# titus-leistner/mmlf

Measured on AMD Instinct MI355X. Metric: 96x96 EPI patches/sec fwd+bwd, bs=512, higher is better.
Workload: dtype f32 via 2 x f16 operand split (22 significant bits per operand, locally scaled; 3 MFMA passes, f32 accumulate)

## Files before the change

### include/mmlf_hip.h

```cpp
#ifndef MMLF_HIP_H
#define MMLF_HIP_H

#include <stddef.h>
#include <stdint.h>

#ifdef __cplusplus
extern "C" {
#endif

#define MMLF_TILE_POSITIONS 256

const char *mmlf_last_error(void);
#define MMLF_ABI_VERSION 10
int mmlf_abi_version(void);

const char *mmlf_build_info(void);
int mmlf_build_is_ablation(void);
int mmlf_conv_cus(void);

enum { MMLF_AUDIT_IN = 0, MMLF_AUDIT_PACKED = 1, MMLF_AUDIT_BIAS = 2, MMLF_AUDIT_OUT = 3, MMLF_AUDIT_REF = 4,
       MMLF_AUDIT_IN_AMAX = 5, MMLF_AUDIT_OUT_AMAX = 6, MMLF_AUDIT_BN_PARTIAL = 7, MMLF_AUDIT_MASK = 8, MMLF_AUDIT_CONV_N = 9 };
int mmlf_audit_conv_h2(int cs_in, int K, int N, int cs_out, int N_store, int out_shift, int cs_ref, int B, int H, int W,
                       int64_t *ends);
enum { MMLF_AUDIT_WG_IN = 0, MMLF_AUDIT_WG_G = 1, MMLF_AUDIT_WG_GW = 2, MMLF_AUDIT_WG_GB = 3, MMLF_AUDIT_WG_WORKSPACE = 4,
       MMLF_AUDIT_WG_IN_AMAX = 5, MMLF_AUDIT_WG_G_AMAX = 6, MMLF_AUDIT_WGRAD_N = 7 };
int mmlf_audit_wgrad_h2(int cs_in, int Cin, int cs_g, int Cout, int g_shift, int B, int H, int W, int64_t *ends);

int64_t mmlf_grid_alloc_positions(int B, int H, int W);
int64_t mmlf_packed_filter_floats(int K, int N);
int64_t mmlf_wgrad_workspace_floats(int Cin, int Cout, int B, int H, int W);

enum { MMLF_VAR_IDENTITY = 0, MMLF_VAR_TRANSPOSE = 1, MMLF_VAR_TRANSPOSE_FLIPH = 2 };

int mmlf_pack_filter(const float *w_oihw, float *packed, int Cout, int Cin, int variant, int dgrad,
                     void *stream);

int mmlf_conv2x2(const float *in, int cs_in, int K, const float *packed, const float *bias, int N,
                 float *out, int cs_out, int N_store, int out_shift, int vh, int vw,
                 int B, int H, int W, int relu, const float *relu_ref, int cs_ref, void *stream);

int64_t mmlf_packed_filter_split_bytes(int K, int N);
int mmlf_pack_filter_split(const float *w_oihw, void *packed, int Cout, int Cin, int variant, int dgrad,
                           void *stream);
int mmlf_conv2x2_split(const float *in, int cs_in, int K, const void *packed, const float *bias, int N,
                       float *out, int cs_out, int N_store, int out_shift, int vh, int vw,
                       int B, int H, int W, int relu, const float *relu_ref, int cs_ref, void *stream);
// ... 2 lines not shown
int mmlf_grid_pad_w(void);
int mmlf_grid_pad_h(void);
int mmlf_amax_head(void);
int mmlf_amax_shard_stride(void);
int64_t mmlf_packed_filter_h2_bytes(int K, int N);
int mmlf_pack_filter_h2(const float *w_oihw, void *packed, int Cout, int Cin, int variant, int dgrad, void *stream);
typedef struct mmlf_pack_desc {
    const float *w_oihw;
    void *packed;
    int32_t Cout, Cin, variant, dgrad;
    int32_t col0;
    int32_t np;
} mmlf_pack_desc;
int mmlf_packed_filter_h2_columns(int N);
int mmlf_pack_filters_h2(const mmlf_pack_desc *table, int n, int total_columns, void *stream);
int mmlf_conv2x2_h2(const float *in, int cs_in, int K, const void *packed, const float *bias, int N,
                    float *out, int cs_out, int N_store, int out_shift, int vh, int vw,
                    int B, int H, int W, int relu, const float *relu_ref, int cs_ref,
                    const float *in_amax , float *out_amax ,
                    double *bn_partial ,
                    uint32_t *relu_mask_out , const uint32_t *relu_mask_in , void *stream);
int64_t mmlf_relu_mask_words(int B, int H, int W);
int mmlf_conv2x2_blocks(int K, int N, int B, int H, int W);

int64_t mmlf_conv2x2_thin_workspace_floats(int B, int H, int W);
int mmlf_conv2x2_thin(const float *in, int cs_in, int K, const float *w_oihw, const float *bias, int N,
                      float *out, int cs_out, int out_shift, int vh, int vw, int B, int H, int W, int relu,
                      int variant, float *workspace, float *out_amax, void *stream);
int64_t mmlf_conv2x2_wgrad_thin_workspace_floats(int Cin);
int mmlf_conv2x2_wgrad_thin(const float *in, int cs_in, int Cin, const float *g, int cs_g, int Cout, int g_shift,
                            float *gw_oihw, float *gb, int variant, int accumulate, float *workspace,
                            int B, int H, int W, void *stream);

int mmlf_conv2x2_wgrad(const float *in, int cs_in, int Cin, const float *g, int cs_g, int Cout,
                       int g_shift, float *gw_oihw, float *gb, int variant, int accumulate,
                       float *workspace, int B, int H, int W, void *stream);

int mmlf_conv2x2_wgrad_split(const float *in, int cs_in, int Cin, const float *g, int cs_g, int Cout,
                             int g_shift, float *gw_oihw, float *gb, int variant, int accumulate,
                             float *workspace, int B, int H, int W, void *stream);

int mmlf_conv2x2_wgrad_h2(const float *in, int cs_in, int Cin, const float *g, int cs_g, int Cout,
                          int g_shift, float *gw_oihw, float *gb, int variant, int accumulate,
                          float *workspace, int B, int H, int W, const float *in_amax, const float *g_amax,
                          void *stream);

int mmlf_bn_stats_train(const float *z, int cs, int C, const float *gamma, const float *beta,
                        float *running_mean, float *running_var, double momentum, double eps,
                        float *save_mean, float *save_invstd, float *scale, float *shift,
                        double *partial, int nblocks, int B, int H, int W, void *stream);
int mmlf_bn_coeffs_eval(const float *gamma, const float *beta, const float *running_mean,
                        const float *running_var, double eps, float *scale, float *shift, int C,
                        void *stream);
int mmlf_fold_bn_eval(const float *w_oihw, const float *bias, const float *scale, const float *shift,
                      float *w_out, float *bias_out, int Cout, int Cin, void *stream);
int mmlf_bn_stats_finalize(const double *partial, int nblocks, int C, const float *gamma, const float *beta,
                           float *running_mean, float *running_var, double momentum, double eps,
                           float *save_mean, float *save_invstd, float *scale, float *shift,
                           int B, int H, int W, void *stream);
int mmlf_bn_apply_relu(const float *z, int cs_z, int C, const float *scale, const float *shift,
                       float *y, int cs_y, int c_off, int C_store, int B, int H, int W,
                       float *amax_out , void *stream);
int mmlf_bn_apply_relu4(const float *const z[4], int cs_z, int C, const float *const scale[4],
                        const float *const shift[4], float *y, int cs_y, int B, int H, int W,
                        float *amax_out , void *stream);
int mmlf_bn_bwd_reduce(const float *gy, int cs_gy, int c_off, const float *z, int cs_z, int C,
                       const float *scale, const float *shift, const float *gamma,
                       const float *save_mean, const float *save_invstd,
                       float *dgamma, float *dbeta, int accumulate, float *coef,
                       double *partial, int nblocks, int B, int H, int W, void *stream);
int mmlf_bn_bwd_apply(const float *gy, int cs_gy, int c_off, const float *z, int cs_z, int C,
                      const float *scale, const float *shift, const float *save_mean,
                      const float *coef, float *dz, int cs_dz, int B, int H, int W,
                      float *amax_out , void *stream);
int mmlf_relu_bwd_slice(const float *src, int cs_src, int c_off, const float *ref, int cs_ref, int ref_off, int C,
                        float *dst, int cs_dst, int B, int H, int W,
// ... 77 lines not shown
```

### mmlf_amd/csrc/wgrad.hip

```cpp
#include "conv_device.h"
#include "wgrad_map.h"
#include "row_walk.h"

#ifdef MMLF_BOUNDS_DEBUG
int mmlf_oob_counts_wgrad(unsigned long long *host8, int reset)
{
    if (hipMemcpyFromSymbol(host8, HIP_SYMBOL(g_mmlf_oob), sizeof(unsigned long long) * 8) != hipSuccess) return 1;
    if (reset) {
        const unsigned long long z[8] = {};
        if (hipMemcpyToSymbol(HIP_SYMBOL(g_mmlf_oob), z, sizeof(z)) != hipSuccess) return 1;
    }
    return 0;
}
#endif

struct WgradArgs {
    const float *in;
    const float *g;
    float *part;
    long long NQpad;
    int cs_in, cin, cs_g, g_shift, P, nsplit, nslice, chunks_per_split, nchunks;
    int items;
    int g_cols;
    const float *in_amax, *g_amax;
// ... 845 lines not shown
    WgradPlan p;
    if (!wgrad_plan(0, Cin, Cout, -1, p) || B <= 0 || H <= 0 || W <= 0) return -1;
    return p.scales_off + 2 * (make_grid(B, H, W).NQpad / WG_KQ) + 4;
}

template <int KS, int NT>
static int launch_wgrad_f32(const WgradArgs &a, hipStream_t st)
{
    using S = WgradF32Shape<KS>;
    const dim3 grid(wgrad_grid_blocks(a.nslice, a.nsplit)), block(64 * S::WAVES);
    if constexpr (KS == 2) hipLaunchKernelGGL(wgrad4tap_kernel<NT>, grid, block, S::lds_bytes(NT), st, a);
    else hipLaunchKernelGGL(wgrad9tap_kernel<NT>, grid, block, S::lds_bytes(NT), st, a);
    return mmlf_launch_status(KS == 2 ? "mmlf_conv2x2_wgrad" : "mmlf_conv3x3_wgrad");
}

template <int MB, int NB, int PL>
static int launch_wgrad16(const WgradArgs &a, hipStream_t st)
{
    constexpr size_t lds = 2 * PL * 34 * 32 * (MB | 1) + PL * WG_KQ * 32 * (NB | 1);
    static PerDeviceOnce attr_once;
    if (attr_once.run([] { return mmlf_allow_lds(reinterpret_cast<const void *>(wgrad4tap_x6n_kernel<MB, NB, PL>), lds, "mmlf_conv2x2_wgrad_split"); }))
        return 1;
    hipLaunchKernelGGL((wgrad4tap_x6n_kernel<MB, NB, PL>), dim3(wgrad_grid_blocks(a.nslice, a.nsplit)), dim3(256), lds, st, a);
    return mmlf_launch_status("mmlf_conv2x2_wgrad_split");
}

static bool wgrad_persist()
{
    static const bool on = [] { const char *e = getenv("MMLF_WGRAD_PERSIST"); return !e || atoi(e) != 0; }();
    return on;
}

template <int PL>
static int launch_wgrad_wide(const WgradArgs &a, hipStream_t st)
{
    constexpr size_t lds = 2 * (2 * PL * 34 * 32 * (3 | 1) + PL * WG_KQ * 32 * (18 | 1));
    static PerDeviceOnce attr_once;
    if (attr_once.run([] { return mmlf_allow_lds(reinterpret_cast<const void *>(wgrad4tap_x6w_kernel<3, 9, PL>), lds, "mmlf_conv2x2_wgrad_split(wide)"); }))
        return 1;
    hipLaunchKernelGGL((wgrad4tap_x6w_kernel<3, 9, PL>), dim3(wgrad_wide_grid(a.items, device_cus(), wgrad_persist())), dim3(512), lds, st, a);
    return mmlf_launch_status("mmlf_conv2x2_wgrad_split");
}

template <int PL>
static int launch_wgrad_split(const Wgrad16Cfg &c, const WgradArgs &a, hipStream_t st)
{
    switch (10 * c.mb + c.nb) {
    case 22: return launch_wgrad16<2, 2, PL>(a, st);
    case 52: return launch_wgrad16<5, 2, PL>(a, st);
    case 25: return launch_wgrad16<2, 5, PL>(a, st);
    case 55: return launch_wgrad16<5, 5, PL>(a, st);
    case 28: return launch_wgrad16<2, 8, PL>(a, st);
    case 38: return launch_wgrad16<3, 8, PL>(a, st);
    default: return launch_wgrad_wide<PL>(a, st);
    }
}

static WgradArgs wgrad_args(const float *in, int cs_in, int Cin, const float *g, int cs_g, int g_shift, float *workspace,
                            const Grid &gr, long long alloc, long long part_floats)
{
    WgradArgs a = {};
    a.in = in; a.g = g; a.part = workspace; a.NQpad = gr.NQpad;
    a.cs_in = cs_in; a.cin = Cin; a.cs_g = a.g_cols = cs_g; a.g_shift = g_shift; a.P = gr.P;
    a.in_bytes = alloc * cs_in * 4; a.g_bytes = alloc * cs_g * 4;
    a.part_floats = part_floats;
    a.nchunks = (int)(gr.NQpad / WG_KQ);
    return a;
}
static void wgrad_set_grid(WgradArgs &a, int nslice, int nsplit)
{
    a.nslice = nslice;
    a.nsplit = nsplit;
    a.chunks_per_split = (a.nchunks + nsplit - 1) / nsplit;
    a.items = (int)wgrad_grid_blocks(nslice, nsplit);
}

template <int KS>
static int wgrad_reduce(const WgradArgs &a, float *gw, float *gb, int Cin, int Cout, int CIP, int NP, int variant,
                        int accumulate, hipStream_t st)
{
    const int total = KS * KS * (Cin + 1) * Cout;
    hipLaunchKernelGGL(wgrad_reduce_kernel<KS * KS>, dim3((total + 255) / 256), dim3(256), 0, st, a.part, gw, gb, Cin, Cout,
                       CIP, NP, a.nsplit, variant, accumulate);
    return mmlf_launch_status(KS == 2 ? "mmlf_conv2x2_wgrad(reduce)" : "mmlf_conv3x3_wgrad(reduce)");
}

template <int KS>
static int wgrad_run_block(WgradArgs &a, const WgradBlock &k, int planes, float *gw, float *gb, int Cin, int variant,
                           int accumulate, hipStream_t st)
{
    wgrad_set_grid(a, k.nslice, k.nsplit);
    int rc = 1;
    if constexpr (KS == 2) {
        if (!k.nt) rc = planes == 3 ? launch_wgrad_split<3>(k.cfg, a, st) : launch_wgrad_split<2>(k.cfg, a, st);
    }
    if (k.nt) switch (k.nt) {
    case 1: rc = launch_wgrad_f32<KS, 1>(a, st); break;
    case 3: rc = launch_wgrad_f32<KS, 3>(a, st); break;
    case 4: rc = launch_wgrad_f32<KS, 4>(a, st); break;
    default: rc = launch_wgrad_f32<KS, 9>(a, st); break;
    }
    if (rc) return rc;
    return wgrad_reduce<KS>(a, gw, gb, Cin, k.cout, k.CIP, k.NP, variant, accumulate, st);
}

static int wgrad_impl(const float *in, int cs_in, int Cin, const float *g, int cs_g, int Cout, int g_shift,
                      float *gw, float *gb, int variant, int accumulate, float *workspace, int B, int H, int W,
                      void *stream, int planes, const float *in_amax = nullptr, const float *g_amax = nullptr);

extern "C" int mmlf_conv2x2_wgrad(const float *in, int cs_in, int Cin, const float *g, int cs_g, int Cout,
                                  int g_shift, float *gw, float *gb, int variant, int accumulate,
                                  float *workspace, int B, int H, int W, void *stream)
{
    return wgrad_impl(in, cs_in, Cin, g, cs_g, Cout, g_shift, gw, gb, variant, accumulate, workspace, B, H, W,
                      stream, 0);
}

extern "C" int mmlf_conv2x2_wgrad_split(const float *in, int cs_in, int Cin, const float *g, int cs_g, int Cout,
                                        int g_shift, float *gw, float *gb, int variant, int accumulate,
                                        float *workspace, int B, int H, int W, void *stream)
{
    return wgrad_impl(in, cs_in, Cin, g, cs_g, Cout, g_shift, gw, gb, variant, accumulate, workspace, B, H, W,
                      stream, 3);
}

extern "C" int mmlf_conv2x2_wgrad_h2(const float *in, int cs_in, int Cin, const float *g, int cs_g, int Cout,
                                     int g_shift, float *gw, float *gb, int variant, int accumulate,
                                     float *workspace, int B, int H, int W, const float *in_amax,
                                     const float *g_amax, void *stream)
{
    MMLF_CHECK_ARG(in_amax && g_amax, "mmlf_conv2x2_wgrad_h2: the f16 split needs max |in| and max |g|");
    return wgrad_impl(in, cs_in, Cin, g, cs_g, Cout, g_shift, gw, gb, variant, accumulate, workspace, B, H, W,
                      stream, 2, in_amax, g_amax);
}

static int wgrad_impl(const float *in, int cs_in, int Cin, const float *g, int cs_g, int Cout, int g_shift,
                      float *gw, float *gb, int variant, int accumulate, float *workspace, int B, int H, int W,
                      void *stream, int planes, const float *in_amax, const float *g_amax)
{
    MMLF_CHECK_ARG(in && g && (gw || gb) && workspace, "mmlf_conv2x2_wgrad: null pointer");
    MMLF_CHECK_ARG(cs_in % 4 == 0 && cs_g % 4 == 0, "mmlf_conv2x2_wgrad: strides must be multiples of 4");
    MMLF_CHECK_ARG(Cin > 0 && Cin <= cs_in && Cout > 0 && Cout <= cs_g, "mmlf_conv2x2_wgrad: channels vs strides");
    MMLF_CHECK_ARG(Cout <= WGRAD_MAX_COUT_WIDE, "mmlf_conv2x2_wgrad: Cout=%d not supported (max %d)", Cout, WGRAD_MAX_COUT_WIDE);
    MMLF_CHECK_ARG(variant >= 0 && variant <= 2, "mmlf_conv2x2_wgrad: bad variant");
    Grid gr = make_grid(B, H, W);
    MMLF_CHECK_ARG(g_shift >= 0 && g_shift <= gr.P + 1, "mmlf_conv2x2_wgrad: g_shift=%d", g_shift);
    WgradPlan p;
    MMLF_CHECK_ARG(wgrad_plan(planes, Cin, Cout, gr.NQpad / WG_KQ, p), "mmlf_conv2x2_wgrad: no launch plan");
    WgradArgs a = wgrad_args(in, cs_in, Cin, g, cs_g, g_shift, workspace, gr, grid_alloc_positions(gr), p.scales_off);
    a.in_amax = in_amax; a.g_amax = g_amax;
    hipStream_t st = (hipStream_t)stream;
    if (!gw)
        return bias_grad_only("mmlf_conv2x2_wgrad", g, cs_g, Cout, g_shift, gb, accumulate, workspace, p.scales_off, gr, st);
    if (planes == 2) {
        MMLF_CHECK_ARG(gr.NQpad + 2 * gr.P + 64 < (1ll << 31), "mmlf_conv2x2_wgrad_h2: batch x image too large");
        ChunkScaleArgs ca;
        ca.in_amax = in_amax; ca.g_amax = g_amax; ca.out = workspace + p.scales_off;
        ca.NQ = gr.NQ; ca.nchunks = a.nchunks; ca.P = gr.P; ca.g_shift = g_shift;
        ca.nrows = (int)amax_rows(gr);
        ca.divP = make_magic((unsigned)gr.P);
        hipLaunchKernelGGL(wgrad_chunk_scales_kernel, dim3((a.nchunks + 255) / 256), dim3(256), 0, st, ca);
        a.chunk_scales = ca.out;
    }
    const WgradArgs whole = a;
    for (int b = 0; b < p.nblocks; ++b) {
        const int c0 = p.blk[b].c0;
        a = whole;
        a.g = g + c0; a.g_cols = cs_g - c0; a.g_bytes = whole.g_bytes - 4ll * c0;
        const int rc = wgrad_run_block<2>(a, p.blk[b], planes, gw + (size_t)c0 * Cin * 4, gb ? gb + c0 : nullptr, Cin, variant,
                                          accumulate, st);
        if (rc) return rc;
    }
    return 0;
}

__global__ __launch_bounds__(256) void thin_wgrad_kernel(ThinArgs a)
{
    const int lane = threadIdx.x & 63;
    const long long wave = __builtin_amdgcn_readfirstlane((int)(blockIdx.x * 4 + (threadIdx.x >> 6)));
    const long long nwaves = gridDim.x * 4ll;
    float acc[2][4][THIN_MAXN][4];
#pragma unroll
    for (int h = 0; h < 2; ++h)
#pragma unroll
        for (int t = 0; t < 4; ++t)
#pragma unroll
            for (int o = 0; o < THIN_MAXN; ++o)
#pragma unroll
                for (int k = 0; k < 4; ++k) acc[h][t][o][k] = 0.f;
    float gsum[THIN_MAXN] = {0.f, 0.f};
    const bool first = 4 * lane < a.cs_in, second = 256 + 4 * lane < a.cs_in;
    const int offs[4] = {0, 1, a.P, a.P + 1};
    constexpr int U = 4;
    for (long long p0 = U * wave; p0 < a.npos; p0 += U * nwaves) {
        float4 x0[U], x1[U];
        float gt[U][4][THIN_MAXN];
#pragma unroll
        for (int u = 0; u < U; ++u) {
            const long long p = p0 + u < a.npos ? p0 + u : a.npos - 1;
            const float *row = a.in + (size_t)p * a.cs_in;
            x0[u] = first ? *reinterpret_cast<const float4 *>(row + 4 * lane) : make_float4(0.f, 0.f, 0.f, 0.f);
            x1[u] = second ? *reinterpret_cast<const float4 *>(row + 256 + 4 * lane) : make_float4(0.f, 0.f, 0.f, 0.f);
#pragma unroll
// ... 140 lines not shown
```

### mmlf_amd/csrc/wgrad_map.h

```cpp
#pragma once

__host__ __device__ __forceinline__ bool wgrad_block_map(int b, int nslice, int nsplit, int &slice, int &split)
{
    const int x = b & 7, j = b >> 3;
    const int reg = (nsplit >> 3) * nslice;
    if (j < reg) {
        slice = j % nslice;
        split = (j / nslice) * 8 + x;
        return true;
    }
    const int left = (nsplit & 7) * nslice, per = (left + 7) >> 3;
    const int m = x * per + (j - reg);
    slice = m % nslice;
    split = (nsplit & ~7) + m / nslice;
    return m < left;
}

static inline unsigned wgrad_grid_blocks(int nslice, int nsplit)
{
    return 8u * (unsigned)((nsplit >> 3) * nslice + ((nsplit & 7) * nslice + 7) / 8);
}

static inline void wgrad_wide_splits(int Cin, long long nchunks, int cus, int &nslice, int &nsplit)
{
    nslice = (Cin + 1 + 47) / 48;
    if (cus > 256 || nchunks < 0) cus = 256;
    const int one_round = cus / nslice, three_rounds = (768 / nslice + 7) / 8 * 8;
    nsplit = nchunks < 0 ? (one_round > three_rounds ? one_round : three_rounds)
                         : (nchunks >= 42 * 1024 ? three_rounds : one_round);
    if (nsplit < 8) nsplit = 8;
}

static inline unsigned wgrad_wide_grid(int items, int cus, bool persist)
{
    if (!persist) return (unsigned)items;
    int resident = cus / 8 * 8;
    if (resident < 8) resident = 8;
    return (unsigned)(items < resident ? items : resident);
}
```

### mmlf_amd/engine.py

```python
import contextlib
import ctypes
import os
import threading
from collections import namedtuple

import torch

from . import _lib
from ._lib import call, check, ptr

VAR_IDENTITY, VAR_TRANSPOSE, VAR_TRANSPOSE_FLIPH = 0, 1, 2
BN_BLOCKS = 1024
LOSS_BLOCKS = 1024


MAX_WIDTH = {2: 512, 3: 288}
MAX_OC = 288
MAX_OVERLAP_WIDTH = 288


def cs_of(c):
    return (c + 7) // 8 * 8


# ... 168 lines not shown
def _toc(events, tag, flops, nbytes):
    events[1].record()
    PROFILE.append((tag, flops, events[0], events[1], nbytes))


@contextlib.contextmanager
def _timed(tag, flops, nbytes):
    events = _tic()
    yield
    _toc(events, tag, flops, nbytes)


_UNTIMED = contextlib.nullcontext()


def _amax_of(geo, t, cs):
    a = getattr(t, 'absmax', None)
    if a is None:
        return geo.amax_of(t, cs)
    if CHECK_ABSMAX:
        true = geo.amax_of(t, cs)
        c = geo.amax_canonical(a)
        exact = geo.P >= 32
        bad = (c != true) if exact else (c < true)
        bad[0] = c[0] != true[0]
        if bool(bad.any()):
            k = int(bad.nonzero()[0])
            raise AssertionError(f'amax entry {k} holds {float(c[k])!r}, true max |x| is {float(true[k])!r}')
    return a


CHECK_ABSMAX = bool(os.environ.get('MMLF_CHECK_ABSMAX'))
OVERLAP_WGRAD = os.environ.get('MMLF_OVERLAP_WGRAD', '1') not in ('', '0')


CHECK_EXTENTS = bool(os.environ.get('MMLF_CHECK_EXTENTS'))
EXTENT_CHECKS = 0


def _audit(entry, scalars, n_ends, kind, have):
    global EXTENT_CHECKS
    ends = (ctypes.c_int64 * n_ends)()
    call(entry, *scalars, ends)
    for name, (k, t, off) in have.items():
        if t is None:
            continue
        got = t.untyped_storage().nbytes() - t.storage_offset() * t.element_size() - 4 * off
        if ends[k] > got:
            raise RuntimeError(f'MMLF_CHECK_EXTENTS: {kind}: the launch may touch {ends[k]} bytes behind `{name}`, '
                               f'the tensor has {got}')
    EXTENT_CHECKS += 1


def relu_bwd_slice(geo, src, cs_src, c_off, ref, cs_ref, ref_off, C, dst, cs_dst):
    amax = getattr(dst, 'absmax', None)
    if CHECK_EXTENTS:
        _audit('mmlf_audit_relu_bwd_slice', (cs_src, c_off, cs_ref, ref_off, C, cs_dst, geo.B, geo.H, geo.W), 4,
               f'relu_bwd_slice C={C} {cs_src}+{c_off} B={geo.B} {geo.H}x{geo.W}',
               {'src': (0, src, 0), 'ref': (1, ref, 0), 'dst': (2, dst, 0), 'amax': (3, amax, 0)})
    call('mmlf_relu_bwd_slice', ptr(src), cs_src, c_off, ptr(ref), cs_ref, ref_off, C, ptr(dst), cs_dst, geo.B, geo.H, geo.W,
         ptr(amax), _lib.stream_ptr())


THIN_MAX_N, THIN_MIN_K = 2, 64


def wgrad(geo, x, cs_in, cin, g, cs_g, cout, g_shift, gw, gb, variant, workspace, side=False):
    if cout <= THIN_MAX_N and cin >= THIN_MIN_K and cs_in <= 512:
        ws = _Workspace.get(x.device).scratch('thin_wgrad', int(_lib.load().mmlf_conv2x2_wgrad_thin_workspace_floats(cin)), side)
        call('mmlf_conv2x2_wgrad_thin', ptr(x), cs_in, cin, ptr(g), cs_g, cout, g_shift, ptr(gw), ptr(gb), variant, 1,
             ptr(ws), geo.B, geo.H, geo.W, _lib.stream_ptr())
        return
    args = (ptr(x), cs_in, cin, ptr(g), cs_g, cout, g_shift, ptr(gw), ptr(gb), variant, 1, ptr(workspace),
            geo.B, geo.H, geo.W)
    timed = _UNTIMED
    if PROFILE is not None and cin >= 256 and cout >= 256 and gw is not None:
        vh, vw = (geo.H + 1, geo.W + 1) if g_shift == 0 else (geo.H, geo.W)
        nbytes = 4.0 * geo.B * (cin * (geo.H * geo.W if g_shift == 0 else (geo.H + 1) * (geo.W + 1)) + cout * vh * vw)
        timed = _timed('wgrad_side' if side else 'wgrad', 2.0 * geo.B * vh * vw * cout * 4 * cin, nbytes)
    with timed:
        if CONV_MODE == 'f16x3':
            ax, ag = _amax_of(geo, x, cs_in), _amax_of(geo, g, cs_g)
            if CHECK_EXTENTS:
                _audit('mmlf_audit_wgrad_h2', (cs_in, cin, cs_g, cout, g_shift, geo.B, geo.H, geo.W), 7,
                       f'wgrad {cin}->{cout} B={geo.B} {geo.H}x{geo.W} g_shift={g_shift}',
                       {'in': (0, x, 0), 'g': (1, g, 0), 'gw': (2, gw, 0), 'gb': (3, gb, 0), 'workspace': (4, workspace, 0),
                        'in_amax': (5, ax, 0), 'g_amax': (6, ag, 0)})
            call('mmlf_conv2x2_wgrad_h2', *args, ptr(ax), ptr(ag), _lib.stream_ptr())
        else:
            call('mmlf_conv2x2_wgrad_split' if CONV_MODE == 'bf16x6' else 'mmlf_conv2x2_wgrad', *args, _lib.stream_ptr())


def conv(geo, x, cs_in, K, packed, bias, N, out, cs_out, out_shift, vh, vw, relu, ref=None, cs_ref=0,
         n_store=None, out_off=0, bn_partial=None, mask_out=None, mask_in=None, w_master=None, variant=0):
    aout = getattr(out, 'absmax', None)
    if (w_master is not None and N <= THIN_MAX_N and K >= THIN_MIN_K and cs_in <= 512 and ref is None and mask_in is None
            and mask_out is None and bn_partial is None and out_off == 0 and n_store in (None, cs_out)):
        ws = _Workspace.get(x.device).scratch('thin_fwd', int(_lib.load().mmlf_conv2x2_thin_workspace_floats(geo.B, geo.H, geo.W)))
        call('mmlf_conv2x2_thin', ptr(x), cs_in, K, ptr(w_master), ptr(bias), N, ptr(out), cs_out, out_shift, vh, vw,
             geo.B, geo.H, geo.W, int(relu), variant, ptr(ws), ptr(aout), _lib.stream_ptr())
        return
    n_store = cs_out if n_store is None else n_store
    timed = _UNTIMED
    if PROFILE is not None and ((K >= 256 and N >= 256) or (K == N and 64 <= K < 128)):
        nbytes = 4.0 * geo.B * (K * (geo.H * geo.W if out_shift == 0 else (geo.H + 1) * (geo.W + 1)) + N * vh * vw)
        timed = _timed('conv' if K >= 256 else 'conv70', 2.0 * geo.B * vh * vw * N * 4 * K, nbytes)
# ... 67 lines not shown
    def __init__(self, geo, device, p=None, train=False, fold=False, plan=None, packs=None, sites=0, running=True):
        self.geo, self.device, self.p, self.train, self.fold, self.plan, self.running = geo, device, p, train, fold, plan, running
        self.packs, self.tracked, self.deferred, self.concat, self.recs = packs or {}, [], None, None, [None] * sites


class _SideWgrad:
    __slots__ = ('main', 'side', 'pending', 'kept', 'on_done')

    def __init__(self, ws, on_done, enabled):
        self.side = ws.side if enabled else None
        self.main = torch.cuda.current_stream() if self.side is not None else None
        self.pending, self.kept, self.on_done = None, None, on_done

    def takes(self, cin):
        return self.side is not None and 128 <= cin <= MAX_OVERLAP_WIDTH

    def launch(self, key, keep, run):
        ready = self.main.record_event()
        with torch.cuda.stream(self.side):
            self.side.wait_event(ready)
            run()
            self.pending, self.kept = (self.side.record_event(), key), keep

    def settle(self):
        if self.pending is not None:
            self.main.wait_event(self.pending[0])
            if self.on_done:
                self.on_done(self.pending[1])
            self.pending = None

    def done(self, key):
        if self.on_done and (self.pending is None or self.pending[1] != key):
            self.on_done(key)


class BlockPlan:
    LAUNCHES = ('reduce', 'apply', 'wgrad2', 'dgrad2', 'wgrad1', 'dgrad1')
    __slots__ = ('prefix', 'want') + LAUNCHES

    def __init__(self, prefix, want, bn, train, need_dx):
        self.prefix, self.want = prefix, frozenset(want)
        want_bn = bn and bool(self.want & {'3.weight', '3.bias'})
        self.wgrad1 = bool(self.want & {'0.weight', '0.bias'})
        self.wgrad2 = bool(self.want & {'2.weight', '2.bias'})
        self.dgrad1 = bool(need_dx)
        self.dgrad2 = self.wgrad1 or self.dgrad1
        need_dz = self.wgrad2 or self.dgrad2
        self.apply = bool(bn) and need_dz
        self.reduce = bool(bn) and (want_bn or (need_dz and bool(train)))

    def launches(self):
        return [k for k in self.LAUNCHES if getattr(self, k)]

    def __eq__(self, other):
        return isinstance(other, BlockPlan) and all(getattr(self, k) == getattr(other, k) for k in self.__slots__)

    def __repr__(self):
        return f'BlockPlan({self.prefix}: {" ".join(self.launches())}; {sorted(self.want)})'


class Plan:

    def __init__(self, trainable, input_grads, train, fold, streams, out, relu_only):
        self.trainable, self.input_grads, self.train, self.fold = trainable, input_grads, train, fold
        self.streams, self.out = streams, out
        self.stream_live = [any(b is not None for b in blocks) for blocks in streams]
# ... 120 lines not shown
                add(f'{spec.prefix}.0.weight', var, True)
        return _Workspace.get(dev).packed_filters(items)

    def _pack(self, w, var, dgrad):
        return (pack_filter3 if self.ksize == 3 else pack_filter)(w, var, dgrad)

    def _packed(self, tape, name, var, dgrad):
        pk = tape.packs.get((name, var, dgrad))
        return pk if pk is not None else self._pack(tape.p[name], var, dgrad)

    def _f16(self):
        return CONV_MODE == 'f16x3' and self.ksize == 2

    _extent = (lambda geo: (0, geo.H + 1, geo.W + 1), lambda geo: (geo.P + 1, geo.H, geo.W))

    def _conv(self, geo, x, f, out, off=None, stats=None):
        n_store, out_off = (out.cs, 0) if off is None else (f.N, off)
        if self.ksize == 3:
            assert out.mask is None and stats is None and f.master is None, (f, out.mask, stats)
            conv3(geo, x.t, x.cs, f.K, f.packed, f.bias, f.N, out.t, out.cs, out.relu, n_store=n_store, out_off=out_off)
            return
        conv(geo, x.t, x.cs, f.K, f.packed, f.bias, f.N, out.t, out.cs, *self._extent[f.second](geo), out.relu,
             n_store=n_store, out_off=out_off, bn_partial=stats, mask_out=out.mask, w_master=f.master, variant=f.var)

    def _dgrad(self, geo, g, f, dx, x):
        relu = {}
        if x.relu:
            relu = {'mask_in': x.mask} if x.mask is not None and self._f16() else {'ref': x.t, 'cs_ref': x.cs}
        if self.ksize == 3:
            conv3(geo, g.t, g.cs, f.N, f.packed, None, f.K, dx.t, dx.cs, False, **relu)
            return
        conv(geo, g.t, g.cs, f.N, f.packed, None, f.K, dx.t, dx.cs, *self._extent[not f.second](geo), False, **relu)

    def _wgrad(self, geo, f, x, g, into, side=False):
        ws = _Workspace.get(x.t.device).wgrad_ws(geo, f.K, f.N, side=side)
        if self.ksize == 3:
            wgrad3(geo, x.t, x.cs, f.K, g.t, g.cs, f.N, *into, f.var, ws)
        else:
            wgrad(geo, x.t, x.cs, f.K, g.t, g.cs, f.N, geo.P + 1 if f.second else 0, *into, f.var, ws, side=side)

    def _bn_fwd(self, tape, spec, z, rec):
        geo, p, pre, C, sp = tape.geo, tape.p, spec.prefix, spec.cout, _lib.stream_ptr
        coef = torch.empty((2 if z is None else 4) * C, dtype=torch.float32, device=tape.device)
        scale, shift = coef[:C], coef[C:2 * C]
        smean, sinv = (None, None) if z is None else (coef[2 * C:3 * C], coef[3 * C:])
        g, bt, rm, rv = (p[f'{pre}.3.{k}'] for k in ('weight', 'bias', 'running_mean', 'running_var'))
        if tape.train:
            partial = _Workspace.get(tape.device).partial
            moved = (rm, rv) if tape.running else (None, None)
            if self._f16():
                nblk = int(_lib.load().mmlf_conv2x2_blocks(C, C, geo.B, geo.H, geo.W))
                call('mmlf_bn_stats_finalize', ptr(partial), nblk, C, ptr(g), ptr(bt), ptr(moved[0]), ptr(moved[1]),
                     self.momentum, self.eps, ptr(smean), ptr(sinv), ptr(scale), ptr(shift), geo.B, geo.H, geo.W, sp())
            else:
                call('mmlf_bn_stats_train', ptr(z), cs_of(C), C, ptr(g), ptr(bt), ptr(moved[0]), ptr(moved[1]), self.momentum,
                     self.eps, ptr(smean), ptr(sinv), ptr(scale), ptr(shift), ptr(partial), BN_BLOCKS, geo.B, geo.H, geo.W, sp())
            if tape.running:
                tape.tracked.append(p[f'{pre}.3.num_batches_tracked'])
        else:
            call('mmlf_bn_coeffs_eval', ptr(g), ptr(bt), ptr(rm), ptr(rv), self.eps, ptr(scale), ptr(shift), C, sp())
            if rec is not None:
                smean.copy_(rm)
                sinv.copy_(torch.rsqrt(rv.double() + self.eps).float())
                rec.eval = True
        if rec is not None:
            rec.scale, rec.shift, rec.smean, rec.sinv = scale, shift, smean, sinv
        return scale, shift, smean, sinv

    def _block_fwd(self, tape, site, x, dest=None):
        geo, p, dev, spec, var = tape.geo, tape.p, tape.device, site.spec, site.var
        C, cs_mid, pre = spec.cout, cs_of(spec.cout), spec.prefix
        w1, b1, w2, b2 = p[f'{pre}.0.weight'], p[f'{pre}.0.bias'], p[f'{pre}.2.weight'], p[f'{pre}.2.bias']
# ... 101 lines not shown
                counts.setdefault(t.data_ptr(), [t, 0])[1] += 1
            torch._foreach_add_([t for t, _ in counts.values()], [n for _, n in counts.values()])
        out = torch.empty((B, self.oc, H, W), dtype=torch.float32, device=dev)
        call('mmlf_unpack_nchw', ptr(x.t), x.cs, ptr(out), self.oc, B, H, W, _lib.stream_ptr())
        if not (save and any(plan.slices)):
            tape.concat = None
        return out, (tape if save else None)

    def _bn_bwd(self, tape, rec, bp, grads, g, dz):
        geo, p, pre, C = tape.geo, tape.p, rec.spec.prefix, rec.spec.cout
        cs_mid, sp, ws = cs_of(C), _lib.stream_ptr, _Workspace.get(tape.device)
        g3w, g3b = (grads[f'{pre}.{k}'] if k in bp.want else None for k in ('3.weight', '3.bias'))
        coef = None
        if bp.reduce:
            coef = torch.empty(3 * C, dtype=torch.float32, device=tape.device)
            dgb = ws.scratch('bn_dgamma_dbeta', 2 * C) if g3w is None or g3b is None else None
            dgamma, dbeta = (dgb[:C] if g3w is None else g3w), (dgb[C:2 * C] if g3b is None else g3b)
            acc = int(g3w is not None or g3b is not None)
            call('mmlf_bn_bwd_reduce', ptr(g.t), g.cs, g.off, ptr(rec.z), cs_mid, C, ptr(rec.scale), ptr(rec.shift),
                 ptr(p[f'{pre}.3.weight']), ptr(rec.smean), ptr(rec.sinv), ptr(dgamma), ptr(dbeta), acc, ptr(coef),
                 ptr(ws.partial), BN_BLOCKS, geo.B, geo.H, geo.W, sp())
            if rec.eval and bp.apply:
                coef[C:].zero_()
        elif bp.apply:
            assert rec.eval, (pre, bp)
            coef = torch.zeros(3 * C, dtype=torch.float32, device=tape.device)
            coef[:C].copy_((p[f'{pre}.3.weight'].double() * rec.sinv.double()).float())
        if not bp.apply:
            return None, coef
        call('mmlf_bn_bwd_apply', ptr(g.t), g.cs, g.off, ptr(rec.z), cs_mid, C, ptr(rec.scale), ptr(rec.shift),
             ptr(rec.smean), ptr(coef), ptr(dz), cs_mid, geo.B, geo.H, geo.W, ptr(dz.absmax), sp())
        return _Slice(dz, cs_mid, 0), coef

    def _block_bwd(self, tape, rec, bp, grads, g, side=None):
        if rec is None:
            raise ValueError(f'Trunk.backward: the forward pass kept no record of {bp.prefix} (its trainable= / '
                             'input_grads= did not ask for what this backward needs)')
        spec, var, x, y, geo = rec.spec, rec.var, rec.x, rec.y, tape.geo
        C, cs_mid, pre = spec.cout, cs_of(spec.cout), spec.prefix
        assert not bp.want or rec.pk2d is None, 'a frozen forward (BatchNorm folded) has no parameter gradients'
        assert bool(rec.bn) or not (bp.reduce or bp.apply), (pre, bp)
        need_dx = bp.dgrad1
        gw1, gb1, gw2, gb2 = (grads[f'{pre}.{k}'] if k in bp.want else None for k in ('0.weight', '0.bias', '2.weight', '2.bias'))
        conv1, conv2 = _Filter(False, spec.cin, C, var), _Filter(True, C, C, var)
        css = ([cs_mid] if bp.apply else []) + ([cs_mid] if bp.dgrad2 else []) + ([x.cs] if need_dx else [])
        got = geo.bufs(css, tape.device) if css else []
        dy = _Slice(got[1 if bp.apply else 0], cs_mid, 0) if bp.dgrad2 else None
        dx = _Slice(got[-1], x.cs, 0) if need_dx else None
        if rec.bn:
            dz, coef = self._bn_bwd(tape, rec, bp, grads, g, got[0] if bp.apply else None)
        else:
            assert g.off == 0 and g.cs == cs_mid
            dz = g
        if side is not None:
            side.settle()
        if bp.wgrad2:
            self._wgrad(geo, conv2, y, dz, (gw2, gb2))
        if bp.dgrad2:
            pk2d = rec.pk2d if rec.pk2d is not None else self._packed(tape, f'{pre}.2.weight', var, True)
            self._dgrad(geo, dz, conv2._replace(packed=pk2d), dy, y)
        del dz, got
        overlap = side is not None and side.takes(spec.cin) and need_dx and bp.wgrad1
        if bp.wgrad1 and not overlap:
            self._wgrad(geo, conv1, x, dy, (gw1, gb1))
        if need_dx:
            self._dgrad(geo, dy, conv1._replace(packed=self._packed(tape, f'{pre}.0.weight', var, True)), dx, x)
        if overlap:
            side.launch(pre, (x.t, dy.t), lambda: self._wgrad(geo, conv1, x, dy, (gw1, gb1), side=True))
        elif side is not None:
            side.kept = None
        return dx

    def backward(self, p, tape, grad_output, grads, on_done=None, input_grads=None, packed_grads=False):
        geo, dev = tape.geo, tape.device
        check(grad_output, 'grad_output', dev, shape=(geo.B, self.oc, geo.H, geo.W), contiguous=False)
        fplan = tape.plan
        if grads is not None:
            wanted = self._grad_names if fplan is None else [n for n in self._grad_names if n in fplan.trainable]
            self._check_dict('grads', grads, wanted, dev)
        ws = _Workspace.get(dev)
        ws.enter_stream()
        B, H, W = geo.B, geo.H, geo.W
        g = _Slice(geo.buf(cs_of(self.oc), dev), cs_of(self.oc), 0)
        call('mmlf_pack_nchw', ptr(grad_output.contiguous()), self.oc, ptr(g.t), g.cs, B, H, W, ptr(g.t.absmax),
             _lib.stream_ptr())
        want = [bool(w) for w in input_grads] if input_grads is not None else [False] * 4
        assert len(want) == 4
        bplan = self.plan(fplan.trainable if grads is not None else (), want, fplan.train, fplan.fold)
        tape.p = p
        side =_SideWgrad(ws, on_done, OVERLAP_WGRAD and self.ksize == 2)
        dstacks = [None] * 4
        for site in reversed(self.sites):
            rec, tape.recs[site.index] = tape.recs[site.index], None
            bp, s = bplan.of(site), site.chain
            if s == 4:
                if bp is None:
                    g = None
                    side.settle()
                else:
                    g = self._block_bwd(tape, rec, bp, grads, g, side)
                side.done(site.spec.prefix)
                continue
            if site.last:
                if s == 2:
                    side.settle()
                gs = None if g is None else _Slice(g.t, g.cs, s * self.chs)
                if bplan.slices[s]:
                    if tape.concat is None:
                        raise ValueError('Trunk.backward: the forward pass kept no concat buffer for this backward')
                    gs = _Slice(geo.buf(cs_of(self.chs), dev), cs_of(self.chs), 0)
                    relu_bwd_slice(geo, g.t, g.cs, s * self.chs, tape.concat, g.cs, s * self.chs, self.chs, gs.t, gs.cs)
            if bp is not None:
                gs = self._block_bwd(tape, rec, bp, grads, gs)
            if site.k == 0:
                if want[s] and packed_grads:
                    assert gs.off == 0
                    dstacks[s] = (gs.t, gs.cs)
                elif want[s]:
                    dstacks[s] = torch.empty((B, self.views, 3, H, W), dtype=torch.float32, device=dev)
                    call('mmlf_unpack_nchw', ptr(gs.t), gs.cs, ptr(dstacks[s]), 3 * self.views, B, H, W, _lib.stream_ptr())
                if s in (2, 0):
                    side.done('in_net_id' if s == 2 else 'in_net_hv')
        tape.concat = None
        return dstacks
```

### mmlf_amd/train.py

```python
import math
import operator

import torch
import torch.distributed as dist

from . import _lib, dl, loss as loss_mod
from ._lib import call, ptr


def flatten_parameters(model):
    params = list(model.named_parameters())
    dev = params[0][1].device
    total = sum(p.numel() for _, p in params)
    flat = torch.empty(total, dtype=torch.float32, device=dev)
    layout, o = [], 0
    for name, p in params:
        n = p.numel()
        flat[o:o + n].copy_(p.detach().reshape(-1))
        p.data = flat[o:o + n].view_as(p)
        layout.append((name, o, n))
        o += n
    return flat, layout


# ... 339 lines not shown
        parts = [t.chunk(self.micro_batches) for t in tensors]
        if len(parts[0]) == 1:
            return None
        assert all(len(part) == len(parts[0]) for part in parts), [t.shape[0] for t in tensors]
        return list(zip(*parts))

    def _chunked_fwd_bwd(self, fwd_bwd, chunks, gt, mask, den):
        share = self.loss.chunks(len(chunks), self.micro_batches, gt, mask, den)
        losses, saved = [], None
        buffers = list(self.model.buffers()) if fwd_bwd == self._torch_fwd_bwd and self.model.training else []
        for k, chunk in enumerate(chunks):
            share.index = k
            losses.append(fwd_bwd(*chunk, share.den, share))
            if buffers:
                with torch.no_grad():
                    if saved is None:
                        saved = [b.clone() for b in buffers]
                    else:
                        torch._foreach_copy_(buffers, saved)
        return torch.stack(losses).sum()

    def _native_fwd_bwd(self, h, v, i_, d, gt, mask, den, share=None):
        model = self.model
        p = model._tensor_dict()
        with torch.no_grad():
            extra = {} if share is None else {'update_running': share.first(), 'packs': share.packs}
            out, tape = model._trunk.forward(p, [h, v, i_, d], model.training, True, trainable=self.trainable, **extra)
            den = self._den_end(den)
            if share is not None:
                share.den, share.packs = den, tape.packs
            loss, gout = self.loss.native(out, gt, mask, den, share)
            hooked = self.distributed and (share is None or share.last())
            on_done = (lambda key: self.buckets.ready(self.grad, key)) if hooked else None
            model._trunk.backward(p, tape, gout, self._trainable_grads or None, on_done)
        return loss

    def _torch_fwd_bwd(self, h, v, i_, d, gt, mask, den, share=None):
        model = self.model
        if share is None or share.first():
            for _, p in model.named_parameters():
                p.grad = None
        out = model(h, v, i_, d)
        den = self._den_end(den)
        if share is not None:
            share.den = den
        loss = self.loss.torch(out, gt, mask, den, share)
        loss.backward()
        if share is not None and not share.last():
            return loss.detach()
        for name, p in model.named_parameters():
            if p.grad is not None:
                self._grads[name].copy_(p.grad)
            p.grad = None
        return loss.detach()

    def _adam(self, lr, grad_scale):
        b1, b2 = self.betas
        t = self.adam_steps
        if self.flat.is_cuda:
            call('mmlf_adam_step', ptr(self.flat), ptr(self.grad), ptr(self.exp_avg), ptr(self.exp_avg_sq),
                 self.flat.numel(), lr, b1, b2, self.eps, t, grad_scale, _lib.stream_ptr())
            return
        with torch.no_grad():
            g = self.grad * grad_scale
            self.exp_avg.lerp_(g, 1 - b1)
            self.exp_avg_sq.mul_(b2).addcmul_(g, g, value=1 - b2)
            bc1, bc2 = 1 - b1 ** t, 1 - b2 ** t
# ... 24 lines not shown
```

Before: 1145.

## Defer chain-4 wgrads to side stream with a CU budget, overlapping the trunk backward

Weight-gradient launches for the first blocks of the shared chain-4 trunk are collected during backward. They are then replayed together on the side stream once the block's dgrad is issued, overlapping with the later backward work. A new flags field carries a CU budget that caps the persistent wide-wgrad grid, so the deferred kernels leave CUs free for the main stream. This adds stream/event synchronisation and a changed ABI, and only turns on in non-distributed training above a batch-size threshold, where the chosen budget may starve or oversubscribe either stream.

```diff
diff --git a/include/mmlf_hip.h b/include/mmlf_hip.h
--- a/include/mmlf_hip.h
+++ b/include/mmlf_hip.h
@@ -11,7 +11,7 @@
 #define MMLF_TILE_POSITIONS 256
 
 const char *mmlf_last_error(void);
-#define MMLF_ABI_VERSION 10
+#define MMLF_ABI_VERSION 11
 int mmlf_abi_version(void);
 
 const char *mmlf_build_info(void);
@@ -80,16 +80,20 @@
                             float *gw_oihw, float *gb, int variant, int accumulate, float *workspace,
                             int B, int H, int W, void *stream);
 
+#define MMLF_WGRAD_ACCUMULATE 1
+#define MMLF_WGRAD_BUDGET_SHIFT 8
+#define MMLF_WGRAD_BUDGET_MASK 0x00ffff00
+#define MMLF_WGRAD_BUDGET(cus) (((cus) << MMLF_WGRAD_BUDGET_SHIFT) & MMLF_WGRAD_BUDGET_MASK)
 int mmlf_conv2x2_wgrad(const float *in, int cs_in, int Cin, const float *g, int cs_g, int Cout,
-                       int g_shift, float *gw_oihw, float *gb, int variant, int accumulate,
+                       int g_shift, float *gw_oihw, float *gb, int variant, int flags,
                        float *workspace, int B, int H, int W, void *stream);
 
 int mmlf_conv2x2_wgrad_split(const float *in, int cs_in, int Cin, const float *g, int cs_g, int Cout,
-                             int g_shift, float *gw_oihw, float *gb, int variant, int accumulate,
+                             int g_shift, float *gw_oihw, float *gb, int variant, int flags,
                              float *workspace, int B, int H, int W, void *stream);
 
 int mmlf_conv2x2_wgrad_h2(const float *in, int cs_in, int Cin, const float *g, int cs_g, int Cout,
-                          int g_shift, float *gw_oihw, float *gb, int variant, int accumulate,
+                          int g_shift, float *gw_oihw, float *gb, int variant, int flags,
                           float *workspace, int B, int H, int W, const float *in_amax, const float *g_amax,
                           void *stream);
 
diff --git a/mmlf_amd/csrc/wgrad.hip b/mmlf_amd/csrc/wgrad.hip
--- a/mmlf_amd/csrc/wgrad.hip
+++ b/mmlf_amd/csrc/wgrad.hip
@@ -901,18 +901,18 @@
 }
 
 template <int PL>
-static int launch_wgrad_wide(const WgradArgs &a, hipStream_t st)
+static int launch_wgrad_wide(const WgradArgs &a, int budget, hipStream_t st)
 {
     constexpr size_t lds = 2 * (2 * PL * 34 * 32 * (3 | 1) + PL * WG_KQ * 32 * (18 | 1));
     static PerDeviceOnce attr_once;
     if (attr_once.run([] { return mmlf_allow_lds(reinterpret_cast<const void *>(wgrad4tap_x6w_kernel<3, 9, PL>), lds, "mmlf_conv2x2_wgrad_split(wide)"); }))
         return 1;
-    hipLaunchKernelGGL((wgrad4tap_x6w_kernel<3, 9, PL>), dim3(wgrad_wide_grid(a.items, device_cus(), wgrad_persist())), dim3(512), lds, st, a);
+    hipLaunchKernelGGL((wgrad4tap_x6w_kernel<3, 9, PL>), dim3(wgrad_wide_grid(a.items, wgrad_wide_budget_cus(device_cus(), budget), wgrad_persist())), dim3(512), lds, st, a);
     return mmlf_launch_status("mmlf_conv2x2_wgrad_split");
 }
 
 template <int PL>
-static int launch_wgrad_split(const Wgrad16Cfg &c, const WgradArgs &a, hipStream_t st)
+static int launch_wgrad_split(const Wgrad16Cfg &c, const WgradArgs &a, int budget, hipStream_t st)
 {
     switch (10 * c.mb + c.nb) {
     case 22: return launch_wgrad16<2, 2, PL>(a, st);
@@ -921,7 +921,7 @@
     case 55: return launch_wgrad16<5, 5, PL>(a, st);
     case 28: return launch_wgrad16<2, 8, PL>(a, st);
     case 38: return launch_wgrad16<3, 8, PL>(a, st);
-    default: return launch_wgrad_wide<PL>(a, st);
+    default: return launch_wgrad_wide<PL>(a, budget, st);
     }
 }
 
@@ -956,12 +956,12 @@
 
 template <int KS>
 static int wgrad_run_block(WgradArgs &a, const WgradBlock &k, int planes, float *gw, float *gb, int Cin, int variant,
-                           int accumulate, hipStream_t st)
+                           int accumulate, hipStream_t st, int budget = 0)
 {
     wgrad_set_grid(a, k.nslice, k.nsplit);
     int rc = 1;
     if constexpr (KS == 2) {
-        if (!k.nt) rc = planes == 3 ? launch_wgrad_split<3>(k.cfg, a, st) : launch_wgrad_split<2>(k.cfg, a, st);
+        if (!k.nt) rc = planes == 3 ? launch_wgrad_split<3>(k.cfg, a, budget, st) : launch_wgrad_split<2>(k.cfg, a, budget, st);
     }
     if (k.nt) switch (k.nt) {
     case 1: rc = launch_wgrad_f32<KS, 1>(a, st); break;
@@ -974,40 +974,43 @@
 }
 
 static int wgrad_impl(const float *in, int cs_in, int Cin, const float *g, int cs_g, int Cout, int g_shift,
-                      float *gw, float *gb, int variant, int accumulate, float *workspace, int B, int H, int W,
+                      float *gw, float *gb, int variant, int flags, float *workspace, int B, int H, int W,
                       void *stream, int planes, const float *in_amax = nullptr, const float *g_amax = nullptr);
 
 extern "C" int mmlf_conv2x2_wgrad(const float *in, int cs_in, int Cin, const float *g, int cs_g, int Cout,
-                                  int g_shift, float *gw, float *gb, int variant, int accumulate,
+                                  int g_shift, float *gw, float *gb, int variant, int flags,
                                   float *workspace, int B, int H, int W, void *stream)
 {
-    return wgrad_impl(in, cs_in, Cin, g, cs_g, Cout, g_shift, gw, gb, variant, accumulate, workspace, B, H, W,
+    return wgrad_impl(in, cs_in, Cin, g, cs_g, Cout, g_shift, gw, gb, variant, flags, workspace, B, H, W,
                       stream, 0);
 }
 
 extern "C" int mmlf_conv2x2_wgrad_split(const float *in, int cs_in, int Cin, const float *g, int cs_g, int Cout,
-                                        int g_shift, float *gw, float *gb, int variant, int accumulate,
+                                        int g_shift, float *gw, float *gb, int variant, int flags,
                                         float *workspace, int B, int H, int W, void *stream)
 {
-    return wgrad_impl(in, cs_in, Cin, g, cs_g, Cout, g_shift, gw, gb, variant, accumulate, workspace, B, H, W,
+    return wgrad_impl(in, cs_in, Cin, g, cs_g, Cout, g_shift, gw, gb, variant, flags, workspace, B, H, W,
                       stream, 3);
 }
 
 extern "C" int mmlf_conv2x2_wgrad_h2(const float *in, int cs_in, int Cin, const float *g, int cs_g, int Cout,
-                                     int g_shift, float *gw, float *gb, int variant, int accumulate,
+                                     int g_shift, float *gw, float *gb, int variant, int flags,
                                      float *workspace, int B, int H, int W, const float *in_amax,
                                      const float *g_amax, void *stream)
 {
     MMLF_CHECK_ARG(in_amax && g_amax, "mmlf_conv2x2_wgrad_h2: the f16 split needs max |in| and max |g|");
-    return wgrad_impl(in, cs_in, Cin, g, cs_g, Cout, g_shift, gw, gb, variant, accumulate, workspace, B, H, W,
+    return wgrad_impl(in, cs_in, Cin, g, cs_g, Cout, g_shift, gw, gb, variant, flags, workspace, B, H, W,
                       stream, 2, in_amax, g_amax);
 }
 
 static int wgrad_impl(const float *in, int cs_in, int Cin, const float *g, int cs_g, int Cout, int g_shift,
-                      float *gw, float *gb, int variant, int accumulate, float *workspace, int B, int H, int W,
+                      float *gw, float *gb, int variant, int flags, float *workspace, int B, int H, int W,
                       void *stream, int planes, const float *in_amax, const float *g_amax)
 {
     MMLF_CHECK_ARG(in && g && (gw || gb) && workspace, "mmlf_conv2x2_wgrad: null pointer");
+    MMLF_CHECK_ARG((flags & ~(MMLF_WGRAD_ACCUMULATE | MMLF_WGRAD_BUDGET_MASK)) == 0, "mmlf_conv2x2_wgrad: unknown bits in flags=0x%x", flags);
+    const int accumulate = flags & MMLF_WGRAD_ACCUMULATE, budget = (flags & MMLF_WGRAD_BUDGET_MASK) >> MMLF_WGRAD_BUDGET_SHIFT;
+    MMLF_CHECK_ARG(budget % 8 == 0, "mmlf_conv2x2_wgrad: budget=%d is no multiple of 8", budget);
     MMLF_CHECK_ARG(cs_in % 4 == 0 && cs_g % 4 == 0, "mmlf_conv2x2_wgrad: strides must be multiples of 4");
     MMLF_CHECK_ARG(Cin > 0 && Cin <= cs_in && Cout > 0 && Cout <= cs_g, "mmlf_conv2x2_wgrad: channels vs strides");
     MMLF_CHECK_ARG(Cout <= WGRAD_MAX_COUT_WIDE, "mmlf_conv2x2_wgrad: Cout=%d not supported (max %d)", Cout, WGRAD_MAX_COUT_WIDE);
@@ -1037,7 +1040,7 @@
         a = whole;
         a.g = g + c0; a.g_cols = cs_g - c0; a.g_bytes = whole.g_bytes - 4ll * c0;
         const int rc = wgrad_run_block<2>(a, p.blk[b], planes, gw + (size_t)c0 * Cin * 4, gb ? gb + c0 : nullptr, Cin, variant,
-                                          accumulate, st);
+                                          accumulate, st, budget);
         if (rc) return rc;
     }
     return 0;
diff --git a/mmlf_amd/csrc/wgrad_map.h b/mmlf_amd/csrc/wgrad_map.h
--- a/mmlf_amd/csrc/wgrad_map.h
+++ b/mmlf_amd/csrc/wgrad_map.h
@@ -38,3 +38,8 @@
     if (resident < 8) resident = 8;
     return (unsigned)(items < resident ? items : resident);
 }
+
+static inline int wgrad_wide_budget_cus(int cus, int budget)
+{
+    return budget > 0 && budget < cus ? budget : cus;
+}
diff --git a/mmlf_amd/engine.py b/mmlf_amd/engine.py
--- a/mmlf_amd/engine.py
+++ b/mmlf_amd/engine.py
@@ -224,6 +224,9 @@
 
 CHECK_ABSMAX = bool(os.environ.get('MMLF_CHECK_ABSMAX'))
 OVERLAP_WGRAD = os.environ.get('MMLF_OVERLAP_WGRAD', '1') not in ('', '0')
+DEFER_WGRAD = int(os.environ.get('MMLF_DEFER_WGRAD', '4') or 0)
+DEFER_WGRAD_CUS = int(os.environ.get('MMLF_DEFER_WGRAD_CUS', '') or 128)
+DEFER_WGRAD_FORCE = os.environ.get('MMLF_DEFER_WGRAD_FORCE', '0') not in ('', '0')
 
 
 CHECK_EXTENTS = bool(os.environ.get('MMLF_CHECK_EXTENTS'))
@@ -257,13 +260,13 @@
 THIN_MAX_N, THIN_MIN_K = 2, 64
 
 
-def wgrad(geo, x, cs_in, cin, g, cs_g, cout, g_shift, gw, gb, variant, workspace, side=False):
+def wgrad(geo, x, cs_in, cin, g, cs_g, cout, g_shift, gw, gb, variant, workspace, side=False, budget=0):
     if cout <= THIN_MAX_N and cin >= THIN_MIN_K and cs_in <= 512:
         ws = _Workspace.get(x.device).scratch('thin_wgrad', int(_lib.load().mmlf_conv2x2_wgrad_thin_workspace_floats(cin)), side)
         call('mmlf_conv2x2_wgrad_thin', ptr(x), cs_in, cin, ptr(g), cs_g, cout, g_shift, ptr(gw), ptr(gb), variant, 1,
              ptr(ws), geo.B, geo.H, geo.W, _lib.stream_ptr())
         return
-    args = (ptr(x), cs_in, cin, ptr(g), cs_g, cout, g_shift, ptr(gw), ptr(gb), variant, 1, ptr(workspace),
+    args = (ptr(x), cs_in, cin, ptr(g), cs_g, cout, g_shift, ptr(gw), ptr(gb), variant, 1 | budget << 8, ptr(workspace),
             geo.B, geo.H, geo.W)
     timed = _UNTIMED
     if PROFILE is not None and cin >= 256 and cout >= 256 and gw is not None:
@@ -397,6 +400,47 @@
     def done(self, key):
         if self.on_done and (self.pending is None or self.pending[1] != key):
             self.on_done(key)
+
+
+def wgrad_three_rounds(geo):
+    return int(_lib.load().mmlf_relu_mask_words(geo.B, geo.H, geo.W)) // 4096 * 8 >= 42 * 1024
+
+
+class _Deferred:
+    __slots__ = ('side', 'blocks', 'cus', 'held', 'end')
+
+    def __init__(self, side, geo, enabled):
+        self.side, self.cus, self.held, self.end = side, DEFER_WGRAD_CUS, [], None
+        on = (enabled and DEFER_WGRAD > 0 and side.side is not None and side.on_done is None
+              and CONV_MODE in ('f16x3', 'bf16x6'))
+        if on and not DEFER_WGRAD_FORCE:
+            on = wgrad_three_rounds(geo)
+        if on and (self.cus <= 0 or self.cus % 8):
+            raise ValueError(f'MMLF_DEFER_WGRAD_CUS={self.cus}: a positive multiple of 8 is required')
+        self.blocks = DEFER_WGRAD if on else 0
+
+    def takes(self, site, width):
+        return site.chain == 4 and site.k < self.blocks and self.side.takes(width)
+
+    def add(self, keep, run):
+        self.held.append((keep, run))
+
+    def flush(self):
+        if not self.held or self.end is not None:
+            return
+        side = self.side
+        ready = side.main.record_event()
+        with torch.cuda.stream(side.side):
+            side.side.wait_event(ready)
+            for _, run in self.held:
+                run(self.cus)
+            self.end = side.side.record_event()
+
+    def finish(self):
+        self.flush()
+        if self.end is not None:
+            self.side.main.wait_event(self.end)
+        self.held, self.end = [], None
 
 
 class BlockPlan:
@@ -583,12 +627,12 @@
             return
         conv(geo, g.t, g.cs, f.N, f.packed, None, f.K, dx.t, dx.cs, *self._extent[not f.second](geo), False, **relu)
 
-    def _wgrad(self, geo, f, x, g, into, side=False):
+    def _wgrad(self, geo, f, x, g, into, side=False, budget=0):
         ws = _Workspace.get(x.t.device).wgrad_ws(geo, f.K, f.N, side=side)
         if self.ksize == 3:
             wgrad3(geo, x.t, x.cs, f.K, g.t, g.cs, f.N, *into, f.var, ws)
         else:
-            wgrad(geo, x.t, x.cs, f.K, g.t, g.cs, f.N, geo.P + 1 if f.second else 0, *into, f.var, ws, side=side)
+            wgrad(geo, x.t, x.cs, f.K, g.t, g.cs, f.N, geo.P + 1 if f.second else 0, *into, f.var, ws, side=side, budget=budget)
 
     def _bn_fwd(self, tape, spec, z, rec):
         geo, p, pre, C, sp = tape.geo, tape.p, spec.prefix, spec.cout, _lib.stream_ptr
@@ -756,7 +800,7 @@
              ptr(rec.smean), ptr(coef), ptr(dz), cs_mid, geo.B, geo.H, geo.W, ptr(dz.absmax), sp())
         return _Slice(dz, cs_mid, 0), coef
 
-    def _block_bwd(self, tape, rec, bp, grads, g, side=None):
+    def _block_bwd(self, tape, rec, bp, grads, g, side=None, defer=None, first=False):
         if rec is None:
             raise ValueError(f'Trunk.backward: the forward pass kept no record of {bp.prefix} (its trainable= / '
                              'input_grads= did not ask for what this backward needs)')
@@ -778,14 +822,20 @@
             dz = g
         if side is not None:
             side.settle()
-        if bp.wgrad2:
+        if bp.wgrad2 and defer is not None and gw2 is not None:
+            defer.add((y.t, dz.t), lambda cus, dz=dz: self._wgrad(geo, conv2, y, dz, (gw2, gb2), side=True, budget=cus))
+        elif bp.wgrad2:
             self._wgrad(geo, conv2, y, dz, (gw2, gb2))
         if bp.dgrad2:
             pk2d = rec.pk2d if rec.pk2d is not None else self._packed(tape, f'{pre}.2.weight', var, True)
             self._dgrad(geo, dz, conv2._replace(packed=pk2d), dy, y)
         del dz, got
         overlap = side is not None and side.takes(spec.cin) and need_dx and bp.wgrad1
-        if bp.wgrad1 and not overlap:
+        last = defer is not None and first
+        if bp.wgrad1 and last and side.takes(spec.cin) and gw1 is not None:
+            defer.add((x.t, dy.t), lambda cus: self._wgrad(geo, conv1, x, dy, (gw1, gb1), side=True, budget=cus))
+            overlap = False
+        elif bp.wgrad1 and not overlap:
             self._wgrad(geo, conv1, x, dy, (gw1, gb1))
         if need_dx:
             self._dgrad(geo, dy, conv1._replace(packed=self._packed(tape, f'{pre}.0.weight', var, True)), dx, x)
@@ -793,9 +843,11 @@
             side.launch(pre, (x.t, dy.t), lambda: self._wgrad(geo, conv1, x, dy, (gw1, gb1), side=True))
         elif side is not None:
             side.kept = None
+        if last:
+            defer.flush()
         return dx
 
-    def backward(self, p, tape, grad_output, grads, on_done=None, input_grads=None, packed_grads=False):
+    def backward(self, p, tape, grad_output, grads, on_done=None, input_grads=None, packed_grads=False, defer_wgrad=False):
         geo, dev = tape.geo, tape.device
         check(grad_output, 'grad_output', dev, shape=(geo.B, self.oc, geo.H, geo.W), contiguous=False)
         fplan = tape.plan
@@ -813,6 +865,7 @@
         bplan = self.plan(fplan.trainable if grads is not None else (), want, fplan.train, fplan.fold)
         tape.p = p
         side =_SideWgrad(ws, on_done, OVERLAP_WGRAD and self.ksize == 2)
+        defer = _Deferred(side, geo, defer_wgrad and any(bplan.of(s) is not None for s in self.sites if s.chain < 4))
         dstacks = [None] * 4
         for site in reversed(self.sites):
             rec, tape.recs[site.index] = tape.recs[site.index], None
@@ -821,8 +874,10 @@
                 if bp is None:
                     g = None
                     side.settle()
+                    defer.flush()
                 else:
-                    g = self._block_bwd(tape, rec, bp, grads, g, side)
+                    g = self._block_bwd(tape, rec, bp, grads, g, side, defer if defer.takes(site, site.spec.cout) else None,
+                                        site.k == 0)
                 side.done(site.spec.prefix)
                 continue
             if site.last:
@@ -845,5 +900,6 @@
                     call('mmlf_unpack_nchw', ptr(gs.t), gs.cs, ptr(dstacks[s]), 3 * self.views, B, H, W, _lib.stream_ptr())
                 if s in (2, 0):
                     side.done('in_net_id' if s == 2 else 'in_net_hv')
+        defer.finish()
         tape.concat = None
         return dstacks
diff --git a/mmlf_amd/train.py b/mmlf_amd/train.py
--- a/mmlf_amd/train.py
+++ b/mmlf_amd/train.py
@@ -395,7 +395,7 @@
             loss, gout = self.loss.native(out, gt, mask, den, share)
             hooked = self.distributed and (share is None or share.last())
             on_done = (lambda key: self.buckets.ready(self.grad, key)) if hooked else None
-            model._trunk.backward(p, tape, gout, self._trainable_grads or None, on_done)
+            model._trunk.backward(p, tape, gout, self._trainable_grads or None, on_done, defer_wgrad=not self.distributed)
         return loss
 
     def _torch_fwd_bwd(self, h, v, i_, d, gt, mask, den, share=None):
```

After: 1157 (median of 6 runs). About the same (+1.0%).
